# lean-dojo/ReProver

Hardware: NVIDIA H100
Metric: premises encoded/sec (reindex_corpus, ByT5-small, seq_len<=512) (higher is better)
Workload: dtype bf16

## Files before the change

### reprover_b200/csrc/rpx_encoder.cu

```cuda
#include <math.h>

#include <new>
#include <vector>

#include "rpx_gemm_launch.cuh"
#include "rpx_kernels.cuh"

namespace rpx {

namespace {

constexpr int kBlockN = 128;

struct LayerW {
  const __nv_bfloat16* qkv;
  const __nv_bfloat16* o;
  const __nv_bfloat16* wi;
  const __nv_bfloat16* wo;
};

struct ProfRec {
  int cls;
  cudaEvent_t a, b;
};
// ... 27 lines not shown
  const float* bias_lut = nullptr;
  std::vector<rpx::LayerW> layers;
  float* debug_hidden = nullptr;
  bool profiling = false;
  std::vector<rpx::ProfRec> prof_pending;
  std::vector<cudaEvent_t> event_pool;
  float prof_ms[RPX_N_KERNEL_CLASSES] = {0};
  int64_t prof_launches[RPX_N_KERNEL_CLASSES] = {0};
  std::vector<int32_t> h_cu_tokens;
  std::vector<int32_t> h_lens;
};

namespace rpx {

namespace {

struct PackedLayout {
  size_t emb, final_ln, bias_lut, bucket_tmp, layer0, layer_stride, qkv, o, wi, wo, total;
};

PackedLayout packed_layout(const rpx_t5_config& c) {
  PackedLayout L{};
  const size_t D = c.d_model, inner = (size_t)c.num_heads * c.d_kv, F = c.d_ff;
  size_t off = 0;
  auto take = [&](size_t bytes) {
    size_t o = off;
    off = align_up(off + bytes, 256);
    return o;
  };
  L.emb = take((size_t)c.vocab_size * D * 4);
  L.final_ln = take(D * 4);
  L.bias_lut = take((size_t)c.num_heads * (2 * c.rel_max_distance + 1) * 4);
  L.bucket_tmp = take((size_t)(2 * c.rel_max_distance + 1) * 4);
  L.layer0 = off;
  L.qkv = 0;
  size_t lo = 0;
  auto ltake = [&](size_t bytes) {
    size_t o = lo;
    lo = align_up(lo + bytes, 256);
    return o;
  };
  L.qkv = ltake(3 * inner * D * 2);
  L.o = ltake(D * inner * 2);
  L.wi = ltake(2 * F * D * 2);
  L.wo = ltake(D * F * 2);
  L.layer_stride = lo;
  L.total = L.layer0 + lo * (size_t)c.num_layers;
  return L;
}

int validate_cfg(const rpx_t5_config* c) {
  RPX_REQUIRE(c != nullptr, RPX_ERR_INVALID, "config is null");
  RPX_REQUIRE(c->d_kv == 64, RPX_ERR_UNSUPPORTED, "d_kv=%d: only 64 is implemented", c->d_kv);
  RPX_REQUIRE(c->d_model % 64 == 0 && c->d_model > 0, RPX_ERR_UNSUPPORTED, "d_model=%d must be a multiple of 64", c->d_model);
  RPX_REQUIRE(c->d_ff % 128 == 0 && c->d_ff > 0, RPX_ERR_UNSUPPORTED, "d_ff=%d must be a multiple of 128", c->d_ff);
  RPX_REQUIRE(c->num_heads > 0 && c->num_layers > 0 && c->vocab_size > 0, RPX_ERR_INVALID, "bad config");
  RPX_REQUIRE(c->rel_buckets >= 4 && c->rel_buckets % 4 == 0 && c->rel_max_distance >= c->rel_buckets / 4 &&
                  c->rel_max_distance <= 2048,
              RPX_ERR_UNSUPPORTED, "unsupported relative attention config (%d buckets, max distance %d)",
              c->rel_buckets, c->rel_max_distance);
  return RPX_OK;
}

__global__ void bias_lut_kernel(const float* __restrict__ rel_bias, const int32_t* __restrict__ buckets,
                                float* __restrict__ lut, int n_heads, int width) {
  const int i = blockIdx.x * blockDim.x + threadIdx.x;
  if (i >= n_heads * width) return;
  const int h = i / width, j = i % width;
  lut[i] = rel_bias[buckets[j] * n_heads + h];
}

struct Workspace {
  int32_t* cu_tokens;
  int64_t* cu_bytes;
  int32_t* ids;
  int32_t* lens;
  int32_t* flag;
  float* h32;
  __nv_bfloat16* h16;
  __nv_bfloat16* qkv;
  __nv_bfloat16* attn;
  __nv_bfloat16* ffn;
  float* ssA;
  float* ssB;
  size_t total;
};

Workspace carve(const rpx_encoder* e, uint8_t* base, int64_t T, int64_t S) {
  Workspace w{};
  const size_t D = e->cfg.d_model, inner = e->inner, F = e->cfg.d_ff;
  size_t off = 0;
  auto take = [&](size_t bytes) {
    uint8_t* p = base ? base + off : nullptr;
    off = align_up(off + bytes, 256);
    return p;
  };
  w.cu_tokens = (int32_t*)take((S + 1) * 4);
  w.cu_bytes = (int64_t*)take((S + 1) * 8);
  w.lens = (int32_t*)take((S + 1) * 4);
  w.flag = (int32_t*)take(256);
  w.ids = (int32_t*)take(T * 4);
  w.h32 = (float*)take(T * D * 4);
  w.h16 = (__nv_bfloat16*)take(T * D * 2);
  w.qkv = (__nv_bfloat16*)take(T * 3 * inner * 2);
  w.attn = (__nv_bfloat16*)take(T * inner * 2);
  w.ffn = (__nv_bfloat16*)take(T * F * 2);
  const size_t parts = e->n_parts > e->n_parts_lat ? e->n_parts : e->n_parts_lat;
  w.ssA = (float*)take(parts * T * 4);
  w.ssB = (float*)take(parts * T * 4);
  w.total = off;
  return w;
}

struct Prof {
  rpx_encoder* e;
  cudaStream_t st;
  int cls;
  cudaEvent_t a = nullptr, b = nullptr;
  Prof(rpx_encoder* e_, cudaStream_t st_, int cls_) : e(e_), st(st_), cls(cls_) {
    if (!e->profiling) return;
    a = get();
    b = get();
    cudaEventRecord(a, st);
  }
  ~Prof() {
    if (!e->profiling) return;
    cudaEventRecord(b, st);
    e->prof_pending.push_back({cls, a, b});
  }
  cudaEvent_t get() {
    if (!e->event_pool.empty()) {
      cudaEvent_t ev = e->event_pool.back();
      e->event_pool.pop_back();
      return ev;
    }
    cudaEvent_t ev;
    cudaEventCreate(&ev);
    return ev;
  }
};

constexpr int kLatBlockN = 64;
constexpr int kLatStages = 6;
constexpr int kLatSmallM = 64;
constexpr int kLatSmallStages = 12;
constexpr int kLatSmallMMaxTokens = 384;
constexpr int kPdlMaxTokens = 16384;

struct PdlScope {
  explicit PdlScope(bool on) { set_pdl_scope(on); }
  ~PdlScope() { set_pdl_scope(false); }
};

int ss_parts(int d_model, bool latency) {
  return ceil_div(d_model, latency ? 32 : kBlockN) * (EpiResidual::kWarps / 4);
}


int qkv_gemm(bool latency, int T, const void* A, const void* B, int N, int K, const RowScale& rs, __nv_bfloat16* out,
             const void* prefetch, size_t prefetch_bytes, cudaStream_t st) {
  EpiStoreBF16::Params ep{out, N, rs};
  if (!latency) return launch_gemm<kBlockN, EpiStoreBF16>(A, K, B, K, T, N, K, ep, st);
  if (T <= kLatSmallMMaxTokens)
    return launch_gemm<kLatBlockN, EpiStoreBF16, false, kLatSmallStages, false, kLatSmallM>(A, K, B, K, T, N, K, ep, st, 0,
                                                                                             prefetch, prefetch_bytes);
  return launch_gemm<kLatBlockN, EpiStoreBF16, false, kLatStages>(A, K, B, K, T, N, K, ep, st, 0, prefetch, prefetch_bytes);
}

int residual_gemm(bool latency, int T, const void* A, const void* B, int N, int K, float* h32, __nv_bfloat16* h16,
                  float* ss_out, cudaStream_t st) {
  EpiResidualParams ep{h32, h16, N, ss_out, T};
  if (!latency) return launch_gemm<kBlockN, EpiResidual>(A, K, B, K, T, N, K, ep, st);
  if (T <= kLatSmallMMaxTokens)
    return launch_gemm<kLatBlockN, EpiResidualT<true>, false, kLatSmallStages, false, kLatSmallM>(A, K, B, K, T, N, K, ep, st);
  return launch_gemm<kLatBlockN, EpiResidualT<true>, false, kLatStages>(A, K, B, K, T, N, K, ep, st);
}
int oproj_gemm(bool latency, int T, const void* A, const void* B, int N, int K, float* h32, __nv_bfloat16* h16,
               float* ss_out, cudaStream_t st) {
  return residual_gemm(latency, T, A, B, N, K, h32, h16, ss_out, st);
}
int ffn_down_gemm(bool latency, int T, const void* A, const void* B, int N, int K, float* h32, __nv_bfloat16* h16,
                  float* ss_out, cudaStream_t st) {
  return residual_gemm(latency, T, A, B, N, K, h32, h16, ss_out, st);
}

int ffn_up_gemm(bool latency, int T, const void* A, const void* B, int N, int K, const RowScale& rs,
                __nv_bfloat16* out, cudaStream_t st) {
  RPX_REQUIRE(N % 256 == 0, RPX_ERR_UNSUPPORTED, "ffn-up gemm: N=%d must be a multiple of 256 (2 x d_ff, d_ff %% 128 == 0)", N);
  const int F = N / 2;
  if (!latency) {
    EpiWsGeGLU::Params ep{out, F, rs};
    return launch_gemm_ws<EpiWsGeGLU>(A, K, B, K, T, N, K, ep, st);
  }
  if (T <= kBlockM) {
    EpiGeGLUT<32>::Params ep{out, F, rs};
    return launch_gemm<64, EpiGeGLUT<32>, false, kLatStages, true>(A, K, B, K, T, N, K, ep, st);
  }
  EpiGeGLUT<64>::Params ep{out, F, rs};
  return launch_gemm<128, EpiGeGLUT<64>, false, kGemmStages, true>(A, K, B, K, T, N, K, ep, st);
}

int forward_latency_layer(rpx_encoder* e, const Workspace& ws, const LayerW& w, const void* next_weights,
                          size_t next_bytes, int T, int S, int max_len, cudaStream_t st) {
  const rpx_t5_config& c = e->cfg;
  const int D = c.d_model, inner = e->inner, F = c.d_ff, P = e->n_parts_lat;
  const float inv_d = 1.0f / (float)D;
  {
    Prof p(e, st, 1);
    RPX_TRY(qkv_gemm(true, T, ws.h16, w.qkv, 3 * inner, D, RowScale{ws.ssA, P, T, inv_d, c.ln_eps}, ws.qkv, next_weights,
                     next_bytes, st));
  }
  {
    Prof p(e, st, 2);
    RPX_TRY(launch_t5_attention(ws.qkv, ws.attn, ws.cu_tokens, e->bias_lut, T, S, max_len, c.num_heads, c.d_kv,
                                c.rel_max_distance, st));
  }
  {
    Prof p(e, st, 3);
    RPX_TRY(oproj_gemm(true, T, ws.attn, w.o, D, inner, ws.h32, ws.h16, ws.ssB, st));
  }
  {
    Prof p(e, st, 4);
    RPX_TRY(ffn_up_gemm(true, T, ws.h16, w.wi, 2 * F, D, RowScale{ws.ssB, P, T, inv_d, c.ln_eps}, ws.ffn, st));
  }
  {
    Prof p(e, st, 5);
    RPX_TRY(ffn_down_gemm(true, T, ws.ffn, w.wo, D, F, ws.h32, ws.h16, ws.ssA, st));
  }
  return RPX_OK;
}

int forward(rpx_encoder* e, const Workspace& ws, int T, int S, int max_len, void* d_out, int out_dtype,
            cudaStream_t st) {
  const rpx_t5_config& c = e->cfg;
  const int D = c.d_model, inner = e->inner, F = c.d_ff;
  const bool latency = T <= e->latency_tokens && D % 32 == 0 && (3 * inner) % 32 == 0;
  const int P = latency ? e->n_parts_lat : e->n_parts;
  const float inv_d = 1.0f / (float)D;
  PdlScope pdl_scope(latency || T <= kPdlMaxTokens);
  {
    Prof p(e, st, 0);
    RPX_TRY(launch_embed(ws.ids, e->emb, ws.h32, ws.h16, ws.ssA, T, P, T, D, st));
  }
  auto dump = [&](int slab) -> int {
    if (e->debug_hidden)
      RPX_CUDA_OK(cudaMemcpyAsync(e->debug_hidden + (size_t)slab * T * D, ws.h32, (size_t)T * D * 4,
                                  cudaMemcpyDeviceToDevice, st));
    return RPX_OK;
  };
  RPX_TRY(dump(0));
  for (int l = 0; l < c.num_layers; ++l) {
    const LayerW& w = e->layers[l];
    if (latency) {
      const bool has_next = l + 1 < c.num_layers;
      RPX_TRY(forward_latency_layer(e, ws, w, has_next ? e->layers[l + 1].qkv : nullptr, has_next ? e->layer_bytes : 0, T, S,
                                    max_len, st));
      RPX_TRY(dump(l + 1));
      continue;
    }
    {
      Prof p(e, st, 1);
      RPX_TRY(qkv_gemm(false, T, ws.h16, w.qkv, 3 * inner, D, RowScale{ws.ssA, P, T, inv_d, c.ln_eps}, ws.qkv, nullptr, 0,
                       st));
    }
    {
      Prof p(e, st, 2);
      RPX_TRY(launch_t5_attention(ws.qkv, ws.attn, ws.cu_tokens, e->bias_lut, T, S, max_len, c.num_heads, c.d_kv,
                                  c.rel_max_distance, st));
    }
    {
      Prof p(e, st, 3);
      RPX_TRY(oproj_gemm(false, T, ws.attn, w.o, D, inner, ws.h32, ws.h16, ws.ssB, st));
    }
    {
      Prof p(e, st, 4);
      RPX_TRY(ffn_up_gemm(false, T, ws.h16, w.wi, 2 * F, D, RowScale{ws.ssB, P, T, inv_d, c.ln_eps}, ws.ffn, st));
    }
    {
      Prof p(e, st, 5);
      RPX_TRY(ffn_down_gemm(false, T, ws.ffn, w.wo, D, F, ws.h32, ws.h16, ws.ssA, st));
    }
    RPX_TRY(dump(l + 1));
  }
  {
    Prof p(e, st, 6);
    float* scratch = latency && (size_t)F * 2 >= (size_t)D * 4 ? reinterpret_cast<float*>(ws.ffn) : nullptr;
    RPX_TRY(launch_pool_normalize(ws.h32, ws.ssA, T, P, e->final_ln, ws.cu_tokens, d_out, out_dtype, S, D,
                                  c.ln_eps, st, scratch, max_len));
  }
  return RPX_OK;
}

}
}

using namespace rpx;

extern "C" {

size_t rpx_encoder_packed_bytes(const rpx_t5_config* cfg) {
  if (validate_cfg(cfg) != RPX_OK) return 0;
  return packed_layout(*cfg).total;
}

int rpx_encoder_create(const rpx_t5_config* cfg, const rpx_t5_weights* w, void* d_packed, size_t packed_bytes,
                       void* stream, rpx_encoder** out) {
  RPX_TRY(validate_cfg(cfg));
  RPX_REQUIRE(w && d_packed && out, RPX_ERR_INVALID, "rpx_encoder_create: null argument");
  DeviceInfo dev;
  RPX_TRY(get_device_info(&dev));
  const PackedLayout L = packed_layout(*cfg);
  RPX_REQUIRE(packed_bytes >= L.total, RPX_ERR_WORKSPACE, "packed buffer too small: %zu < %zu", packed_bytes, L.total);
  RPX_REQUIRE((reinterpret_cast<uintptr_t>(d_packed) & 255) == 0, RPX_ERR_INVALID, "packed buffer must be 256-byte aligned");
  cudaStream_t st = static_cast<cudaStream_t>(stream);
  uint8_t* base = static_cast<uint8_t*>(d_packed);
  const int D = cfg->d_model, inner = cfg->num_heads * cfg->d_kv, F = cfg->d_ff;

  rpx_encoder* e = new (std::nothrow) rpx_encoder();
  RPX_REQUIRE(e != nullptr, RPX_ERR_INVALID, "out of host memory");
  e->cfg = *cfg;
  e->inner = inner;
  e->n_parts = ss_parts(D, false);
  e->n_parts_lat = ss_parts(D, true);
  auto fail = [&](int code) {
    delete e;
    return code;
  };
#define TRY_E(expr)                        \
  do {                                     \
    int _s = (expr);                       \
    if (_s != RPX_OK) return fail(_s);     \
  } while (0)
#define CUDA_E(expr)                                                                                   \
  do {                                                                                                 \
    cudaError_t _c = (expr);                                                                           \
    if (_c != cudaSuccess) {                                                                           \
// ... 206 lines not shown
```

### reprover_b200/csrc/rpx_gemm.cuh

```cuda
#pragma once
#include "rpx_ptx.cuh"

namespace rpx {

constexpr int kBlockM = 128;
constexpr int kBlockK = 64;
constexpr int kMmaK = 16;
#ifndef RPX_EPI_WARPS
#define RPX_EPI_WARPS 4
#endif
constexpr int kMmaThreads = 128;
constexpr int kProducerWarp = 4;
constexpr int kEpiWarp0 = 5;
template <class Epi>
constexpr int gemm_threads() { return kMmaThreads + 32 + 32 * Epi::kWarps; }

template <int BLOCK_N, int STAGES, int BM = kBlockM>
struct GemmCfg {
  static_assert(BM == 64 || BM == 128, "tile rows: one or two 64-row wgmma blocks");
  static_assert(BLOCK_N == 64 || BLOCK_N == 128, "wgmma N of a tile: 64 or 128");
  static_assert(2 * STAGES + 2 <= 30, "barrier block holds at most 14 stages");
  static constexpr int kABytes = BM * kBlockK * 2;
  static constexpr int kBBytes = BLOCK_N * kBlockK * 2;
  static constexpr int kStageBytes = kABytes + kBBytes;
// ... 221 lines not shown
      }
      mbar_arrive(tfull);
      tphase ^= 1;
    }
  } else {
    const int lane_grp = (warp - kEpiWarp0) & 3;
    const int lane = threadIdx.x & 31;
    const int row = BM == kBlockM ? lane_grp * 32 + lane : (lane < 16 ? lane_grp * 16 + lane : (1 << 28));
    const int acc_row = BM == kBlockM ? lane_grp * 32 + lane : lane_grp * 16 + (lane & 15);
    const int part = (warp - kEpiWarp0) >> 2;
    pdl_wait();
    Epi epi(ep, smem_extra, lane_grp * 32 + lane, part);
    uint32_t tphase = 0;
    for (int u = unit0; u < num_units; u += unit_step) {
      TileCtx t;
      t.n_blk = unit_n(u);
      t.m_blk = unit_m(u);
      t.m0 = t.m_blk * BM;
      t.rows_per_warp = BM / 4;
      t.n0 = t.n_blk * n_blk_stride * BLOCK_N;
      int n_this = N - t.n0;
      if (n_this > BLOCK_N) n_this = BLOCK_N;
      t.n_cols = n_this;
      t.row = row;
      t.part = part;
      t.split = Epi::kWarps / 4;
      t.M = M;
      t.N = N;
      t.acc = sAcc + acc_row * Cfg::kAccStride;
      {
        const int nu = u + unit_step;
        if (nu < num_units) {
          t.next_m0 = unit_m(nu) * BM;
          t.next_n0 = unit_n(nu) * BLOCK_N;
          t.next_cols = N - t.next_n0 < BLOCK_N ? N - t.next_n0 : BLOCK_N;
        } else {
          t.next_m0 = -1;
          t.next_n0 = 0;
          t.next_cols = 0;
        }
      }
      epi.before_wait(t);
      mbar_wait(tfull, tphase);
      if (threadIdx.x == 32 * kEpiWarp0 && u == unit0) RPX_STAMP(pf, 5);
      epi.tile(t);
      if (threadIdx.x == 32 * kEpiWarp0 && u == unit0) RPX_STAMP(pf, 6);
      mbar_arrive(tempty);
      tphase ^= 1;
    }
    epi.finish();
  }

  __syncthreads();
  if (PAIR) cluster_sync_all();
  if (threadIdx.x == 0) RPX_STAMP(pf, 7);
}


struct RowScale {
  const float* ss_parts;
  int n_parts;
  int part_stride;
  float inv_dim;
  float eps;
  __device__ float get(int m) const {
    if (ss_parts == nullptr) return 1.0f;
    float s = 0.f;
    constexpr int kBatch = 24;
    for (int p = 0; p < n_parts; p += kBatch) {
      float v[kBatch];
#pragma unroll
      for (int j = 0; j < kBatch; ++j) v[j] = p + j < n_parts ? ss_parts[(size_t)(p + j) * part_stride + m] : 0.f;
#pragma unroll
      for (int j = 0; j < kBatch; ++j)
        if (p + j < n_parts) s += v[j];
    }
    return rsqrtf(s * inv_dim + eps);
  }
};

struct EpiStoreF32 {
  struct Params {
    float* C;
    int ldc;
  };
  static constexpr size_t kSmemBytes = 0;
  static constexpr int kWarps = RPX_EPI_WARPS;
  Params p;
  __device__ EpiStoreF32(const Params& p_, uint8_t*, int, int) : p(p_) {}
  __device__ void before_wait(const TileCtx&) {}
  __device__ void tile(const TileCtx& t) {
    const int m = t.m0 + t.row;
    const bool ok = m < t.M;
    for (int c = 32 * t.part; c < t.n_cols; c += 32 * t.split) {
      uint32_t v[32];
      acc_ld32(t.acc + c, v);
      if (ok) {
        float4* dst = reinterpret_cast<float4*>(p.C + (size_t)m * p.ldc + t.n0 + c);
#pragma unroll
        for (int i = 0; i < 8; ++i)
          dst[i] = make_float4(__uint_as_float(v[4 * i]), __uint_as_float(v[4 * i + 1]),
                               __uint_as_float(v[4 * i + 2]), __uint_as_float(v[4 * i + 3]));
      }
    }
  }
  __device__ void finish() {}
};

struct EpiStoreBF16 {
  struct Params {
    __nv_bfloat16* C;
    int ldc;
    RowScale rs;
  };
  static constexpr size_t kSmemBytes = 0;
  static constexpr int kWarps = RPX_EPI_WARPS;
  Params p;
  float rs = 0.f;
  __device__ EpiStoreBF16(const Params& p_, uint8_t*, int, int) : p(p_) {}
  __device__ void before_wait(const TileCtx& t) {
    const int m = t.m0 + t.row;
    rs = m < t.M ? p.rs.get(m) : 0.f;
  }
  __device__ void tile(const TileCtx& t) {
    const int m = t.m0 + t.row;
    const bool ok = m < t.M;
    for (int c = 32 * t.part; c < t.n_cols; c += 32 * t.split) {
      uint32_t v[32];
      acc_ld32(t.acc + c, v);
      if (ok) {
        uint4* dst = reinterpret_cast<uint4*>(p.C + (size_t)m * p.ldc + t.n0 + c);
#pragma unroll
        for (int i = 0; i < 4; ++i) {
          uint4 o;
          o.x = pack_bf16x2(__uint_as_float(v[8 * i + 0]) * rs, __uint_as_float(v[8 * i + 1]) * rs);
          o.y = pack_bf16x2(__uint_as_float(v[8 * i + 2]) * rs, __uint_as_float(v[8 * i + 3]) * rs);
          o.z = pack_bf16x2(__uint_as_float(v[8 * i + 4]) * rs, __uint_as_float(v[8 * i + 5]) * rs);
          o.w = pack_bf16x2(__uint_as_float(v[8 * i + 6]) * rs, __uint_as_float(v[8 * i + 7]) * rs);
          dst[i] = o;
        }
      }
    }
  }
  __device__ void finish() {}
};

struct EpiResidualParams {
  float* h32;
  __nv_bfloat16* h16;
  int ld;
  float* ss_out;
  int ss_stride;
};
template <bool CHUNK_SS>
struct EpiResidualT {
  using Params = EpiResidualParams;
  static constexpr int kWarps = RPX_EPI_WARPS;
  static constexpr size_t kSmemBytes = kWarps * 32 * 32 * sizeof(float);
  Params p;
  float4* stg;
  int lane, grp;
  float4 h[8];
  __device__ EpiResidualT(const Params& p_, uint8_t* smem_extra, int row, int part) : p(p_) {
    lane = row & 31;
    grp = row >> 5;
    stg = reinterpret_cast<float4*>(smem_extra) + (part * 4 + grp) * 32 * 8;
  }
  __device__ __forceinline__ void load_chunk(const TileCtx& t, int c, int row_base, int sub, int col4,
                                             float4 (&hh)[8]) const {
    const size_t col = (size_t)t.n0 + c + col4;
#pragma unroll
    for (int i = 0; i < 8; ++i) {
      const int r = sub + 4 * i, m = row_base + r;
      if (r < t.rows_per_warp && m < t.M) hh[i] = *reinterpret_cast<const float4*>(p.h32 + (size_t)m * p.ld + col);
      else hh[i] = make_float4(0.f, 0.f, 0.f, 0.f);
    }
  }
  __device__ void before_wait(const TileCtx& t) {
    const int c = 32 * t.part;
    if (c < t.n_cols) load_chunk(t, c, t.m0 + grp * t.rows_per_warp, lane >> 3, (lane & 7) * 4, h);
  }
  __device__ void tile(const TileCtx& t) {
    const int sub = lane >> 3;
    const int j4 = lane & 7;
    const int col4 = j4 * 4;
    const int row_base = t.m0 + grp * t.rows_per_warp;
    const int step = 32 * t.split;
    float ss[8];
#pragma unroll
    for (int i = 0; i < 8; ++i) ss[i] = 0.f;
    float4 hn[8];
    int c = 32 * t.part;
    for (; c < t.n_cols; c += step) {
      uint32_t v[32];
      acc_ld32(t.acc + c, v);
      if (c + step < t.n_cols) load_chunk(t, c + step, row_base, sub, col4, hn);
      const size_t col = (size_t)t.n0 + c + col4;
#pragma unroll
      for (int j = 0; j < 8; ++j)
        stg[lane * 8 + (j ^ (lane & 7))] =
            make_float4(__uint_as_float(v[4 * j]), __uint_as_float(v[4 * j + 1]), __uint_as_float(v[4 * j + 2]),
                        __uint_as_float(v[4 * j + 3]));
      __syncwarp();
#pragma unroll
      for (int i = 0; i < 8; ++i) {
        const int r = sub + 4 * i;
        const int m = row_base + r;
        const float4 a = stg[r * 8 + (j4 ^ (r & 7))];
        h[i].x += a.x;
        h[i].y += a.y;
        h[i].z += a.z;
        h[i].w += a.w;
        ss[i] += h[i].x * h[i].x + h[i].y * h[i].y + h[i].z * h[i].z + h[i].w * h[i].w;
        if (r < t.rows_per_warp && m < t.M) {
          *reinterpret_cast<float4*>(p.h32 + (size_t)m * p.ld + col) = h[i];
          *reinterpret_cast<uint2*>(p.h16 + (size_t)m * p.ld + col) =
              make_uint2(pack_bf16x2(h[i].x, h[i].y), pack_bf16x2(h[i].z, h[i].w));
        }
      }
      __syncwarp();
#pragma unroll
      for (int i = 0; i < 8; ++i) h[i] = hn[i];
      if (CHUNK_SS) {
        write_ss(t, ss, row_base, sub, (t.n0 + c) >> 5);
#pragma unroll
        for (int i = 0; i < 8; ++i) ss[i] = 0.f;
      }
    }
    if (!CHUNK_SS) write_ss(t, ss, row_base, sub, t.n_blk * t.split + t.part);
  }
  __device__ __forceinline__ void write_ss(const TileCtx& t, float (&ss)[8], int row_base, int sub, int part_idx) const {
#pragma unroll
    for (int i = 0; i < 8; ++i) {
      float v = ss[i];
      v += __shfl_xor_sync(0xffffffffu, v, 1);
      v += __shfl_xor_sync(0xffffffffu, v, 2);
      v += __shfl_xor_sync(0xffffffffu, v, 4);
      const int r = sub + 4 * i, m = row_base + r;
      if ((lane & 7) == 0 && r < t.rows_per_warp && m < t.M) p.ss_out[(size_t)part_idx * p.ss_stride + m] = v;
    }
  }
  __device__ void finish() {}
};
using EpiResidual = EpiResidualT<false>;

__device__ __forceinline__ float gelu_new(float x) {
  const float k0 = 0.7978845608028654f;
  const float k1 = 0.044715f;
  float u = k0 * (x + k1 * x * x * x);
  float t;
  asm("tanh.approx.f32 %0, %1;" : "=f"(t) : "f"(u));
  return 0.5f * x * (1.0f + t);
}

template <int HALF>
struct EpiGeGLUT {
  struct Params {
    __nv_bfloat16* out;
    int ldo;
    RowScale rs;
  };
  static constexpr size_t kSmemBytes = 0;
  static constexpr int kWarps = RPX_EPI_WARPS;
  Params p;
  float rs = 0.f;
  __device__ EpiGeGLUT(const Params& p_, uint8_t*, int, int) : p(p_) {}
  __device__ void before_wait(const TileCtx& t) {
    const int m = t.m0 + t.row;
    rs = m < t.M ? p.rs.get(m) : 0.f;
  }
  __device__ void tile(const TileCtx& t) {
    const int m = t.m0 + t.row;
    const bool ok = m < t.M;
    for (int c = 32 * t.part; c < HALF; c += 32 * t.split) {
      uint32_t g[32], u[32];
      acc_ld32(t.acc + c, g);
      acc_ld32(t.acc + HALF + c, u);
      if (ok) {
        uint4* dst = reinterpret_cast<uint4*>(p.out + (size_t)m * p.ldo + t.n_blk * HALF + c);
#pragma unroll
        for (int i = 0; i < 4; ++i) {
          float r[8];
#pragma unroll
          for (int j = 0; j < 8; ++j)
            r[j] = gelu_new(__uint_as_float(g[8 * i + j]) * rs) * (__uint_as_float(u[8 * i + j]) * rs);
          uint4 o;
          o.x = pack_bf16x2(r[0], r[1]);
          o.y = pack_bf16x2(r[2], r[3]);
          o.z = pack_bf16x2(r[4], r[5]);
          o.w = pack_bf16x2(r[6], r[7]);
          dst[i] = o;
        }
      }
    }
  }
  __device__ void finish() {}
};

}
```

### reprover_b200/csrc/rpx_gemm_launch.cuh

```cuda
#pragma once
#include "rpx_common.cuh"
#include "rpx_gemm.cuh"
#include "rpx_gemm_ws.cuh"

namespace rpx {

constexpr int kGemmStages = 4;

template <int BLOCK_N, class Epi, bool M_FASTEST = false, int STAGES = kGemmStages, bool SPLIT_B = false, int BM = kBlockM>
int launch_gemm(const void* A, int64_t lda, const void* B, int64_t ldb, int M, int N, int K,
                const typename Epi::Params& ep, cudaStream_t stream, int grid_limit = 0, const void* prefetch_ptr = nullptr,
                size_t prefetch_bytes = 0) {
  using Cfg = GemmCfg<BLOCK_N, STAGES, BM>;
  static_assert(BM == kBlockM || (!M_FASTEST && Epi::kWarps == 4), "64-row tiles: encoder epilogues with one warp per lane group");
  RPX_REQUIRE(M > 0 && N > 0 && K > 0, RPX_ERR_INVALID, "gemm: empty problem M=%d N=%d K=%d", M, N, K);
  RPX_REQUIRE(K % kBlockK == 0, RPX_ERR_UNSUPPORTED, "gemm: K=%d must be a multiple of %d", K, kBlockK);
  RPX_REQUIRE(M_FASTEST || N % 32 == 0, RPX_ERR_UNSUPPORTED, "gemm: N=%d must be a multiple of 32", N);
  DeviceInfo dev;
  RPX_TRY(get_device_info(&dev));
  CUtensorMap tmA, tmB;
  RPX_TRY(make_tmap_bf16_2d(&tmA, A, (uint64_t)M, (uint64_t)K, (uint64_t)lda, BM));
  RPX_TRY(make_tmap_bf16_2d(&tmB, B, (uint64_t)N, (uint64_t)K, (uint64_t)ldb, SPLIT_B ? BLOCK_N / 2 : BLOCK_N));
  RPX_REQUIRE(!SPLIT_B || N % BLOCK_N == 0, RPX_ERR_UNSUPPORTED, "gemm: split-B tiles need N %% %d == 0", BLOCK_N);
  const int tiles_m = ceil_div(M, BM);
  const int tiles_n = ceil_div(N, BLOCK_N);
  const size_t smem = Cfg::smem_bytes(Epi::kSmemBytes);
  RPX_REQUIRE(smem <= dev.smem_optin, RPX_ERR_UNSUPPORTED, "gemm: needs %zu B smem, device allows %zu",
              smem, dev.smem_optin);
  auto kern = gemm_tc_kernel<BLOCK_N, STAGES, Epi, M_FASTEST, SPLIT_B, BM>;
  static thread_local int configured_dev = -1;
  if (configured_dev != dev.device) {
    RPX_CUDA_OK(cudaFuncSetAttribute(kern, cudaFuncAttributeMaxDynamicSharedMemorySize, (int)smem));
    configured_dev = dev.device;
  }
  int grid = tiles_m * tiles_n;
  int cap = grid_limit > 0 ? grid_limit : dev.num_sms;
  if (grid > cap) grid = cap;
  L2Prefetch pf{prefetch_ptr, (uint32_t)prefetch_bytes, grid, next_timeline_slot()};
  if (prefetch_ptr != nullptr && prefetch_bytes > 0 && prefetch_bytes < ((size_t)1 << 32) && grid < dev.num_sms)
    grid = dev.num_sms;
  RPX_CUDA_OK(launch_pdl(kern, dim3(grid), dim3(gemm_threads<Epi>()), smem, stream, pdl_enabled(), tmA, tmB, M, N, K, tiles_m,
                         tiles_n, 1, ep, pf));
  return RPX_OK;
}

template <class Epi>
int launch_gemm_ws(const void* A, int64_t lda, const void* B, int64_t ldb, int M, int N, int K,
                   const typename Epi::Params& ep, cudaStream_t stream) {
  RPX_REQUIRE(M > 0 && N > 0 && K > 0, RPX_ERR_INVALID, "gemm: empty problem M=%d N=%d K=%d", M, N, K);
  RPX_REQUIRE(K % kBlockK == 0, RPX_ERR_UNSUPPORTED, "gemm: K=%d must be a multiple of %d", K, kBlockK);
  RPX_REQUIRE(N % 32 == 0, RPX_ERR_UNSUPPORTED, "gemm: N=%d must be a multiple of 32", N);
  DeviceInfo dev;
  RPX_TRY(get_device_info(&dev));
  CUtensorMap tmA, tmB;
  RPX_TRY(make_tmap_bf16_2d(&tmA, A, (uint64_t)M, (uint64_t)K, (uint64_t)lda, kBlockM));
  RPX_TRY(make_tmap_bf16_2d(&tmB, B, (uint64_t)N, (uint64_t)K, (uint64_t)ldb, kWsBlockN));
  const int tiles_m = ceil_div(M, kBlockM);
  const int tiles_n = ceil_div(N, kWsBlockN);
  const size_t smem = WsCfg::kSmemBytes;
  RPX_REQUIRE(smem <= dev.smem_optin, RPX_ERR_UNSUPPORTED, "gemm: needs %zu B smem, device allows %zu", smem,
              dev.smem_optin);
  auto kern = gemm_ws_kernel<Epi>;
  static thread_local int configured_dev = -1;
  if (configured_dev != dev.device) {
    RPX_CUDA_OK(cudaFuncSetAttribute(kern, cudaFuncAttributeMaxDynamicSharedMemorySize, (int)smem));
    configured_dev = dev.device;
  }
  int grid = tiles_m * tiles_n;
  if (grid > dev.num_sms) grid = dev.num_sms;
  RPX_CUDA_OK(launch_pdl(kern, dim3(grid), dim3(kWsThreads), smem, stream, pdl_enabled(), tmA, tmB, M, N, K, tiles_m,
                         tiles_n, ep));
  return RPX_OK;
}

template <class Epi, int STAGES = kGemmStages>
int launch_gemm_pair(const void* A, int64_t lda, const void* B, int64_t ldb, int M, int N, int K,
                     const typename Epi::Params& ep, cudaStream_t stream) {
  constexpr int BLOCK_N = 128;
  using Cfg = GemmCfg<BLOCK_N, STAGES, kBlockM>;
  RPX_REQUIRE(M > 0 && N > 0 && K > 0, RPX_ERR_INVALID, "gemm: empty problem M=%d N=%d K=%d", M, N, K);
  RPX_REQUIRE(K % kBlockK == 0, RPX_ERR_UNSUPPORTED, "gemm: K=%d must be a multiple of %d", K, kBlockK);
  RPX_REQUIRE(N % 32 == 0, RPX_ERR_UNSUPPORTED, "gemm: N=%d must be a multiple of 32", N);
  DeviceInfo dev;
  RPX_TRY(get_device_info(&dev));
  CUtensorMap tmA, tmB;
  RPX_TRY(make_tmap_bf16_2d(&tmA, A, (uint64_t)M, (uint64_t)K, (uint64_t)lda, kBlockM));
  RPX_TRY(make_tmap_bf16_2d(&tmB, B, (uint64_t)N, (uint64_t)K, (uint64_t)ldb, BLOCK_N / 2));
  const int tiles_m = ceil_div(M, kBlockM);
  const int tiles_n = ceil_div(N, BLOCK_N);
  const size_t smem = Cfg::smem_bytes(Epi::kSmemBytes);
  RPX_REQUIRE(smem <= dev.smem_optin, RPX_ERR_UNSUPPORTED, "gemm: needs %zu B smem, device allows %zu", smem,
              dev.smem_optin);
  auto kern = gemm_tc_kernel<BLOCK_N, STAGES, Epi, false, false, kBlockM, true>;
  static thread_local int configured_dev = -1;
  if (configured_dev != dev.device) {
    RPX_CUDA_OK(cudaFuncSetAttribute(kern, cudaFuncAttributeMaxDynamicSharedMemorySize, (int)smem));
    configured_dev = dev.device;
  }
  int pairs = ceil_div(tiles_m, 2) * tiles_n;
  if (pairs > dev.num_sms / 2) pairs = dev.num_sms / 2;
  cudaLaunchConfig_t cfg{};
  cfg.gridDim = dim3(2 * pairs);
  cfg.blockDim = dim3(gemm_threads<Epi>());
  cfg.dynamicSmemBytes = smem;
  cfg.stream = stream;
  cudaLaunchAttribute at[1];
  at[0].id = cudaLaunchAttributeClusterDimension;
  at[0].val.clusterDim.x = 2;
  at[0].val.clusterDim.y = 1;
  at[0].val.clusterDim.z = 1;
  cfg.attrs = at;
  cfg.numAttrs = 1;
  RPX_CUDA_OK(cudaLaunchKernelEx(&cfg, kern, tmA, tmB, M, N, K, tiles_m, tiles_n, 1, ep,
                                 L2Prefetch{nullptr, 0u, 2 * pairs, next_timeline_slot()}));
  return RPX_OK;
}

}
```

### reprover_b200/csrc/rpx_gemm_ws.cuh

```cuda
#pragma once
#include "rpx_gemm.cuh"

namespace rpx {

constexpr int kWsBlockN = 256;
constexpr int kWsStages = 4;
constexpr int kWsThreads = 384;

struct WsCfg {
  static constexpr int kABytes = kBlockM * kBlockK * 2;
  static constexpr int kBBytes = kWsBlockN * kBlockK * 2;
  static constexpr int kStageBytes = kABytes + kBBytes;
  static constexpr size_t kSmemBytes = (size_t)kWsStages * kStageBytes + 1024 + 256;
};

struct FragCtx {
  int m0, n0;
  int n_blk;
  int n_cols;
  int M, N;
  int r0;
  int q;
};

template <class Epi>
__global__ void __launch_bounds__(kWsThreads, 1)
gemm_ws_kernel(const __grid_constant__ CUtensorMap tmA, const __grid_constant__ CUtensorMap tmB, int M, int N, int K,
               int tiles_m, int tiles_n, typename Epi::Params ep) {
  extern __shared__ uint8_t smem_raw[];
  const uint32_t raw_addr = smem_u32(smem_raw);
  uint8_t* smem = smem_raw + ((1024 - (raw_addr & 1023)) & 1023);
  uint8_t* sA = smem;
  uint8_t* sB = smem + kWsStages * WsCfg::kABytes;
  uint64_t* full = reinterpret_cast<uint64_t*>(smem + kWsStages * WsCfg::kStageBytes);
  uint64_t* empty = full + kWsStages;

  const int warp = threadIdx.x >> 5;
  const int wg = warp >> 2;
  const int num_kb = K / kBlockK;
  const int num_tiles = tiles_m * tiles_n;

  if (threadIdx.x == 0) {
    tma_prefetch_desc(&tmA);
    tma_prefetch_desc(&tmB);
    for (int s = 0; s < kWsStages; ++s) {
      mbar_init(&full[s], 1);
      mbar_init(&empty[s], 2 * 128);
    }
    fence_mbar_init();
  }
  __syncthreads();
  pdl_launch_dependents();
  pdl_wait();

  if (wg == 0) {
    setmaxnreg_dec<40>();
    if (warp == 0 && elect_one()) {
      int stage = 0;
      uint32_t phase = 0;
      for (int t = blockIdx.x; t < num_tiles; t += gridDim.x) {
        const int m_blk = t / tiles_n, n_blk = t % tiles_n;
        for (int kb = 0; kb < num_kb; ++kb) {
          mbar_wait(&empty[stage], phase ^ 1);
          mbar_arrive_expect_tx(&full[stage], WsCfg::kStageBytes);
          tma_load_2d(sA + stage * WsCfg::kABytes, &tmA, &full[stage], kb * kBlockK, m_blk * kBlockM);
          tma_load_2d(sB + stage * WsCfg::kBBytes, &tmB, &full[stage], kb * kBlockK, n_blk * kWsBlockN);
          if (++stage == kWsStages) {
            stage = 0;
            phase ^= 1;
          }
        }
      }
    }
  } else {
    setmaxnreg_inc<232>();
    const int cw = wg - 1;
    const int lane = threadIdx.x & 31;
    Epi epi(ep);
    float acc[128];
    int stage = 0;
    uint32_t phase = 0;
    for (int t = blockIdx.x; t < num_tiles; t += gridDim.x) {
      FragCtx c;
      c.n_blk = t % tiles_n;
      c.m0 = (t / tiles_n) * kBlockM;
      c.n0 = c.n_blk * kWsBlockN;
      c.n_cols = N - c.n0 < kWsBlockN ? N - c.n0 : kWsBlockN;
      c.M = M;
      c.N = N;
      c.r0 = c.m0 + 64 * cw + 16 * (warp & 3) + (lane >> 2);
      c.q = lane & 3;
      int prev = 0;
      for (int kb = 0; kb < num_kb; ++kb) {
        mbar_wait(&full[stage], phase);
        const uint64_t a_desc = make_smem_desc_kmajor_sw128(smem_u32(sA + stage * WsCfg::kABytes)) + 512 * cw;
        const uint64_t b_desc = make_smem_desc_kmajor_sw128(smem_u32(sB + stage * WsCfg::kBBytes));
        wgmma_fence_operand(acc);
        wgmma_fence();
#pragma unroll
        for (int k = 0; k < kBlockK / kMmaK; ++k) wgmma_m64n256k16_ss(acc, a_desc + 2 * k, b_desc + 2 * k, (kb | k) != 0);
        wgmma_commit();
        if (kb == 0) epi.prefetch(c);
        if (kb > 0) {
          wgmma_wait<1>();
          mbar_arrive(&empty[prev]);
        }
        prev = stage;
        if (++stage == kWsStages) {
          stage = 0;
          phase ^= 1;
        }
      }
      wgmma_wait<0>();
      wgmma_fence_operand(acc);
      mbar_arrive(&empty[prev]);
      epi.tile(c, acc);
    }
  }
}


struct EpiWsStoreF32 {
  using Params = EpiStoreF32::Params;
  Params p;
  __device__ explicit EpiWsStoreF32(const Params& p_) : p(p_) {}
  __device__ void prefetch(const FragCtx&) {}
  __device__ void tile(const FragCtx& c, const float (&acc)[128]) {
#pragma unroll
    for (int j = 0; j < 32; ++j) {
      if (8 * j < c.n_cols) {
        float* dst = p.C + (size_t)c.r0 * p.ldc + c.n0 + 8 * j + 2 * c.q;
        if (c.r0 < c.M) *reinterpret_cast<float2*>(dst) = make_float2(acc[4 * j], acc[4 * j + 1]);
        if (c.r0 + 8 < c.M) *reinterpret_cast<float2*>(dst + 8 * (size_t)p.ldc) = make_float2(acc[4 * j + 2], acc[4 * j + 3]);
      }
    }
  }
};

struct EpiWsGeGLU {
  struct Params {
    __nv_bfloat16* out;
    int ldo;
    RowScale rs;
  };
  Params p;
  float rs0 = 0.f, rs1 = 0.f;
  __device__ explicit EpiWsGeGLU(const Params& p_) : p(p_) {}
  __device__ void prefetch(const FragCtx& c) {
    rs0 = c.r0 < c.M ? p.rs.get(c.r0) : 0.f;
    rs1 = c.r0 + 8 < c.M ? p.rs.get(c.r0 + 8) : 0.f;
  }
  __device__ void tile(const FragCtx& c, const float (&acc)[128]) {
    __nv_bfloat16* dst = p.out + (size_t)c.r0 * p.ldo + c.n_blk * (kWsBlockN / 2) + 2 * c.q;
#pragma unroll
    for (int j = 0; j < 16; ++j) {
      const float* g = acc + 4 * j;
      const float* u = acc + 4 * (j + 16);
      if (c.r0 < c.M)
        *reinterpret_cast<uint32_t*>(dst + 8 * j) =
            pack_bf16x2(gelu_new(g[0] * rs0) * (u[0] * rs0), gelu_new(g[1] * rs0) * (u[1] * rs0));
      if (c.r0 + 8 < c.M)
        *reinterpret_cast<uint32_t*>(dst + 8 * (size_t)p.ldo + 8 * j) =
            pack_bf16x2(gelu_new(g[2] * rs1) * (u[2] * rs1), gelu_new(g[3] * rs1) * (u[3] * rs1));
    }
  }
};

}
```

Measured before the change: 3026.

## Route throughput residual GEMMs through warp-specialized kernel with TMA-streamed residual epilogue

Moves the non-latency o-proj and FFN-down residual GEMMs from the classic 128-wide kernel to the persistent warp-specialized 256-wide wgmma kernel. Two idle producer-group warps now stream the fp32 residual in 64x32 chunks via TMA into a small smem ring, and the consumer warpgroups add the accumulator in place, write fp32/bf16 outputs and per-128-column sum-of-squares. Stage count becomes a template parameter, tuned separately per GEMM against the residual buffers. This trades smem and barrier complexity for overlapping residual loads with the MMA mainloop and larger tiles.

```diff
diff --git a/reprover_b200/csrc/rpx_encoder.cu b/reprover_b200/csrc/rpx_encoder.cu
--- a/reprover_b200/csrc/rpx_encoder.cu
+++ b/reprover_b200/csrc/rpx_encoder.cu
@@ -203,9 +203,7 @@
   ~PdlScope() { set_pdl_scope(false); }
 };
 
-int ss_parts(int d_model, bool latency) {
-  return ceil_div(d_model, latency ? 32 : kBlockN) * (EpiResidual::kWarps / 4);
-}
+int ss_parts(int d_model, bool latency) { return ceil_div(d_model, latency ? 32 : 128); }
 
 
 int qkv_gemm(bool latency, int T, const void* A, const void* B, int N, int K, const RowScale& rs, __nv_bfloat16* out,
@@ -218,21 +216,22 @@
   return launch_gemm<kLatBlockN, EpiStoreBF16, false, kLatStages>(A, K, B, K, T, N, K, ep, st, 0, prefetch, prefetch_bytes);
 }
 
+template <int RES_BUFS, int STAGES>
 int residual_gemm(bool latency, int T, const void* A, const void* B, int N, int K, float* h32, __nv_bfloat16* h16,
                   float* ss_out, cudaStream_t st) {
   EpiResidualParams ep{h32, h16, N, ss_out, T};
-  if (!latency) return launch_gemm<kBlockN, EpiResidual>(A, K, B, K, T, N, K, ep, st);
+  if (!latency) return launch_gemm_ws<EpiWsResidual<RES_BUFS>, STAGES>(A, K, B, K, T, N, K, ep, st);
   if (T <= kLatSmallMMaxTokens)
-    return launch_gemm<kLatBlockN, EpiResidualT<true>, false, kLatSmallStages, false, kLatSmallM>(A, K, B, K, T, N, K, ep, st);
-  return launch_gemm<kLatBlockN, EpiResidualT<true>, false, kLatStages>(A, K, B, K, T, N, K, ep, st);
+    return launch_gemm<kLatBlockN, EpiResidualChunkSS, false, kLatSmallStages, false, kLatSmallM>(A, K, B, K, T, N, K, ep, st);
+  return launch_gemm<kLatBlockN, EpiResidualChunkSS, false, kLatStages>(A, K, B, K, T, N, K, ep, st);
 }
 int oproj_gemm(bool latency, int T, const void* A, const void* B, int N, int K, float* h32, __nv_bfloat16* h16,
                float* ss_out, cudaStream_t st) {
-  return residual_gemm(latency, T, A, B, N, K, h32, h16, ss_out, st);
+  return residual_gemm<2, 4>(latency, T, A, B, N, K, h32, h16, ss_out, st);
 }
 int ffn_down_gemm(bool latency, int T, const void* A, const void* B, int N, int K, float* h32, __nv_bfloat16* h16,
                   float* ss_out, cudaStream_t st) {
-  return residual_gemm(latency, T, A, B, N, K, h32, h16, ss_out, st);
+  return residual_gemm<5, 3>(latency, T, A, B, N, K, h32, h16, ss_out, st);
 }
 
 int ffn_up_gemm(bool latency, int T, const void* A, const void* B, int N, int K, const RowScale& rs,
diff --git a/reprover_b200/csrc/rpx_gemm.cuh b/reprover_b200/csrc/rpx_gemm.cuh
--- a/reprover_b200/csrc/rpx_gemm.cuh
+++ b/reprover_b200/csrc/rpx_gemm.cuh
@@ -397,8 +397,7 @@
   float* ss_out;
   int ss_stride;
 };
-template <bool CHUNK_SS>
-struct EpiResidualT {
+struct EpiResidualChunkSS {
   using Params = EpiResidualParams;
   static constexpr int kWarps = RPX_EPI_WARPS;
   static constexpr size_t kSmemBytes = kWarps * 32 * 32 * sizeof(float);
@@ -406,7 +405,7 @@
   float4* stg;
   int lane, grp;
   float4 h[8];
-  __device__ EpiResidualT(const Params& p_, uint8_t* smem_extra, int row, int part) : p(p_) {
+  __device__ EpiResidualChunkSS(const Params& p_, uint8_t* smem_extra, int row, int part) : p(p_) {
     lane = row & 31;
     grp = row >> 5;
     stg = reinterpret_cast<float4*>(smem_extra) + (part * 4 + grp) * 32 * 8;
@@ -466,13 +465,10 @@
       __syncwarp();
 #pragma unroll
       for (int i = 0; i < 8; ++i) h[i] = hn[i];
-      if (CHUNK_SS) {
-        write_ss(t, ss, row_base, sub, (t.n0 + c) >> 5);
-#pragma unroll
-        for (int i = 0; i < 8; ++i) ss[i] = 0.f;
-      }
-    }
-    if (!CHUNK_SS) write_ss(t, ss, row_base, sub, t.n_blk * t.split + t.part);
+      write_ss(t, ss, row_base, sub, (t.n0 + c) >> 5);
+#pragma unroll
+      for (int i = 0; i < 8; ++i) ss[i] = 0.f;
+    }
   }
   __device__ __forceinline__ void write_ss(const TileCtx& t, float (&ss)[8], int row_base, int sub, int part_idx) const {
 #pragma unroll
@@ -487,7 +483,6 @@
   }
   __device__ void finish() {}
 };
-using EpiResidual = EpiResidualT<false>;
 
 __device__ __forceinline__ float gelu_new(float x) {
   const float k0 = 0.7978845608028654f;
diff --git a/reprover_b200/csrc/rpx_gemm_launch.cuh b/reprover_b200/csrc/rpx_gemm_launch.cuh
--- a/reprover_b200/csrc/rpx_gemm_launch.cuh
+++ b/reprover_b200/csrc/rpx_gemm_launch.cuh
@@ -44,7 +44,7 @@
   return RPX_OK;
 }
 
-template <class Epi>
+template <class Epi, int STAGES = 4>
 int launch_gemm_ws(const void* A, int64_t lda, const void* B, int64_t ldb, int M, int N, int K,
                    const typename Epi::Params& ep, cudaStream_t stream) {
   RPX_REQUIRE(M > 0 && N > 0 && K > 0, RPX_ERR_INVALID, "gemm: empty problem M=%d N=%d K=%d", M, N, K);
@@ -52,15 +52,19 @@
   RPX_REQUIRE(N % 32 == 0, RPX_ERR_UNSUPPORTED, "gemm: N=%d must be a multiple of 32", N);
   DeviceInfo dev;
   RPX_TRY(get_device_info(&dev));
-  CUtensorMap tmA, tmB;
+  CUtensorMap tmA, tmB, tmR;
   RPX_TRY(make_tmap_bf16_2d(&tmA, A, (uint64_t)M, (uint64_t)K, (uint64_t)lda, kBlockM));
   RPX_TRY(make_tmap_bf16_2d(&tmB, B, (uint64_t)N, (uint64_t)K, (uint64_t)ldb, kWsBlockN));
+  if constexpr (Epi::kResBufs > 0)
+    RPX_TRY(make_tmap_2d(&tmR, 4, ep.h32, (uint64_t)M, (uint64_t)N, (uint64_t)ep.ld, kResChunkCols, 64, 128));
+  else
+    tmR = tmA;
   const int tiles_m = ceil_div(M, kBlockM);
   const int tiles_n = ceil_div(N, kWsBlockN);
-  const size_t smem = WsCfg::kSmemBytes;
+  const size_t smem = WsCfg<STAGES, Epi::kResBufs>::kSmemBytes;
   RPX_REQUIRE(smem <= dev.smem_optin, RPX_ERR_UNSUPPORTED, "gemm: needs %zu B smem, device allows %zu", smem,
               dev.smem_optin);
-  auto kern = gemm_ws_kernel<Epi>;
+  auto kern = gemm_ws_kernel<Epi, STAGES>;
   static thread_local int configured_dev = -1;
   if (configured_dev != dev.device) {
     RPX_CUDA_OK(cudaFuncSetAttribute(kern, cudaFuncAttributeMaxDynamicSharedMemorySize, (int)smem));
@@ -68,8 +72,8 @@
   }
   int grid = tiles_m * tiles_n;
   if (grid > dev.num_sms) grid = dev.num_sms;
-  RPX_CUDA_OK(launch_pdl(kern, dim3(grid), dim3(kWsThreads), smem, stream, pdl_enabled(), tmA, tmB, M, N, K, tiles_m,
-                         tiles_n, ep));
+  RPX_CUDA_OK(launch_pdl(kern, dim3(grid), dim3(kWsThreads), smem, stream, pdl_enabled(), tmA, tmB, tmR, M, N, K,
+                         tiles_m, tiles_n, ep));
   return RPX_OK;
 }
 
diff --git a/reprover_b200/csrc/rpx_gemm_ws.cuh b/reprover_b200/csrc/rpx_gemm_ws.cuh
--- a/reprover_b200/csrc/rpx_gemm_ws.cuh
+++ b/reprover_b200/csrc/rpx_gemm_ws.cuh
@@ -4,14 +4,19 @@
 namespace rpx {
 
 constexpr int kWsBlockN = 256;
-constexpr int kWsStages = 4;
 constexpr int kWsThreads = 384;
-
+constexpr int kResChunkCols = 32;
+constexpr int kResChunkBytes = 64 * kResChunkCols * 4;
+
+template <int STAGES, int RES_BUFS>
 struct WsCfg {
+  static_assert(2 * STAGES + 4 * RES_BUFS <= 32, "barrier block holds 32 mbarriers");
   static constexpr int kABytes = kBlockM * kBlockK * 2;
   static constexpr int kBBytes = kWsBlockN * kBlockK * 2;
   static constexpr int kStageBytes = kABytes + kBBytes;
-  static constexpr size_t kSmemBytes = (size_t)kWsStages * kStageBytes + 1024 + 256;
+  static constexpr int kRingBytes = STAGES * kStageBytes;
+  static constexpr int kResBytes = 2 * RES_BUFS * kResChunkBytes;
+  static constexpr size_t kSmemBytes = (size_t)kRingBytes + kResBytes + 1024 + 256;
 };
 
 struct FragCtx {
@@ -23,17 +28,29 @@
   int q;
 };
 
-template <class Epi>
+struct ResStream {
+  float* buf;
+  uint64_t* full;
+  uint64_t* empty;
+};
+
+template <class Epi, int STAGES>
 __global__ void __launch_bounds__(kWsThreads, 1)
-gemm_ws_kernel(const __grid_constant__ CUtensorMap tmA, const __grid_constant__ CUtensorMap tmB, int M, int N, int K,
-               int tiles_m, int tiles_n, typename Epi::Params ep) {
+gemm_ws_kernel(const __grid_constant__ CUtensorMap tmA, const __grid_constant__ CUtensorMap tmB,
+               const __grid_constant__ CUtensorMap tmR, int M, int N, int K, int tiles_m, int tiles_n,
+               typename Epi::Params ep) {
+  using Cfg = WsCfg<STAGES, Epi::kResBufs>;
+  constexpr int R = Epi::kResBufs;
   extern __shared__ uint8_t smem_raw[];
   const uint32_t raw_addr = smem_u32(smem_raw);
   uint8_t* smem = smem_raw + ((1024 - (raw_addr & 1023)) & 1023);
   uint8_t* sA = smem;
-  uint8_t* sB = smem + kWsStages * WsCfg::kABytes;
-  uint64_t* full = reinterpret_cast<uint64_t*>(smem + kWsStages * WsCfg::kStageBytes);
-  uint64_t* empty = full + kWsStages;
+  uint8_t* sB = smem + STAGES * Cfg::kABytes;
+  float* sR = reinterpret_cast<float*>(smem + Cfg::kRingBytes);
+  uint64_t* full = reinterpret_cast<uint64_t*>(smem + Cfg::kRingBytes + Cfg::kResBytes);
+  uint64_t* empty = full + STAGES;
+  uint64_t* rfull = empty + STAGES;
+  uint64_t* rempty = rfull + 2 * R;
 
   const int warp = threadIdx.x >> 5;
   const int wg = warp >> 2;
@@ -43,9 +60,14 @@
   if (threadIdx.x == 0) {
     tma_prefetch_desc(&tmA);
     tma_prefetch_desc(&tmB);
-    for (int s = 0; s < kWsStages; ++s) {
+    if (R > 0) tma_prefetch_desc(&tmR);
+    for (int s = 0; s < STAGES; ++s) {
       mbar_init(&full[s], 1);
       mbar_init(&empty[s], 2 * 128);
+    }
+    for (int s = 0; s < 2 * R; ++s) {
+      mbar_init(&rfull[s], 1);
+      mbar_init(&rempty[s], 128);
     }
     fence_mbar_init();
   }
@@ -62,11 +84,33 @@
         const int m_blk = t / tiles_n, n_blk = t % tiles_n;
         for (int kb = 0; kb < num_kb; ++kb) {
           mbar_wait(&empty[stage], phase ^ 1);
-          mbar_arrive_expect_tx(&full[stage], WsCfg::kStageBytes);
-          tma_load_2d(sA + stage * WsCfg::kABytes, &tmA, &full[stage], kb * kBlockK, m_blk * kBlockM);
-          tma_load_2d(sB + stage * WsCfg::kBBytes, &tmB, &full[stage], kb * kBlockK, n_blk * kWsBlockN);
-          if (++stage == kWsStages) {
+          mbar_arrive_expect_tx(&full[stage], Cfg::kStageBytes);
+          tma_load_2d(sA + stage * Cfg::kABytes, &tmA, &full[stage], kb * kBlockK, m_blk * kBlockM);
+          tma_load_2d(sB + stage * Cfg::kBBytes, &tmB, &full[stage], kb * kBlockK, n_blk * kWsBlockN);
+          if (++stage == STAGES) {
             stage = 0;
+            phase ^= 1;
+          }
+        }
+      }
+    } else if (R > 0 && (warp == 1 || warp == 2) && elect_one()) {
+      const int w = warp - 1;
+      float* buf = sR + w * R * (kResChunkBytes / 4);
+      uint64_t* rf = rfull + w * R;
+      uint64_t* re = rempty + w * R;
+      int b = 0;
+      uint32_t phase = 0;
+      for (int t = blockIdx.x; t < num_tiles; t += gridDim.x) {
+        const int row0 = (t / tiles_n) * kBlockM + 64 * w;
+        const int n0 = (t % tiles_n) * kWsBlockN;
+        const int n_cols = N - n0 < kWsBlockN ? N - n0 : kWsBlockN;
+        if (row0 >= M) continue;
+        for (int col = 0; col < n_cols; col += kResChunkCols) {
+          mbar_wait(&re[b], phase ^ 1);
+          mbar_arrive_expect_tx(&rf[b], kResChunkBytes);
+          tma_load_2d(buf + b * (kResChunkBytes / 4), &tmR, &rf[b], n0 + col, row0);
+          if (++b == R) {
+            b = 0;
             phase ^= 1;
           }
         }
@@ -76,7 +120,7 @@
     setmaxnreg_inc<232>();
     const int cw = wg - 1;
     const int lane = threadIdx.x & 31;
-    Epi epi(ep);
+    Epi epi(ep, ResStream{sR + cw * R * (kResChunkBytes / 4), rfull + cw * R, rempty + cw * R});
     float acc[128];
     int stage = 0;
     uint32_t phase = 0;
@@ -93,8 +137,8 @@
       int prev = 0;
       for (int kb = 0; kb < num_kb; ++kb) {
         mbar_wait(&full[stage], phase);
-        const uint64_t a_desc = make_smem_desc_kmajor_sw128(smem_u32(sA + stage * WsCfg::kABytes)) + 512 * cw;
-        const uint64_t b_desc = make_smem_desc_kmajor_sw128(smem_u32(sB + stage * WsCfg::kBBytes));
+        const uint64_t a_desc = make_smem_desc_kmajor_sw128(smem_u32(sA + stage * Cfg::kABytes)) + 512 * cw;
+        const uint64_t b_desc = make_smem_desc_kmajor_sw128(smem_u32(sB + stage * Cfg::kBBytes));
         wgmma_fence_operand(acc);
         wgmma_fence();
 #pragma unroll
@@ -106,7 +150,7 @@
           mbar_arrive(&empty[prev]);
         }
         prev = stage;
-        if (++stage == kWsStages) {
+        if (++stage == STAGES) {
           stage = 0;
           phase ^= 1;
         }
@@ -122,8 +166,9 @@
 
 struct EpiWsStoreF32 {
   using Params = EpiStoreF32::Params;
+  static constexpr int kResBufs = 0;
   Params p;
-  __device__ explicit EpiWsStoreF32(const Params& p_) : p(p_) {}
+  __device__ EpiWsStoreF32(const Params& p_, const ResStream&) : p(p_) {}
   __device__ void prefetch(const FragCtx&) {}
   __device__ void tile(const FragCtx& c, const float (&acc)[128]) {
 #pragma unroll
@@ -143,9 +188,10 @@
     int ldo;
     RowScale rs;
   };
+  static constexpr int kResBufs = 0;
   Params p;
   float rs0 = 0.f, rs1 = 0.f;
-  __device__ explicit EpiWsGeGLU(const Params& p_) : p(p_) {}
+  __device__ EpiWsGeGLU(const Params& p_, const ResStream&) : p(p_) {}
   __device__ void prefetch(const FragCtx& c) {
     rs0 = c.r0 < c.M ? p.rs.get(c.r0) : 0.f;
     rs1 = c.r0 + 8 < c.M ? p.rs.get(c.r0 + 8) : 0.f;
@@ -166,4 +212,79 @@
   }
 };
 
+template <int RES_BUFS>
+struct EpiWsResidual {
+  using Params = EpiResidualParams;
+  static constexpr int kResBufs = RES_BUFS;
+  Params p;
+  ResStream rs;
+  int b = 0;
+  uint32_t phase = 0;
+  __device__ EpiWsResidual(const Params& p_, const ResStream& rs_) : p(p_), rs(rs_) {}
+  __device__ void prefetch(const FragCtx&) {}
+  __device__ void tile(const FragCtx& c, const float (&acc)[128]) {
+    const int lane = threadIdx.x & 31;
+    const int v = (threadIdx.x >> 5) & 3;
+    const int row0 = c.r0 - 16 * v - (lane >> 2);
+    if (row0 >= c.M) return;
+    const int sub = lane >> 3, j4 = lane & 7;
+    float ss[4];
+#pragma unroll
+    for (int k = 0; k < kWsBlockN / kResChunkCols; ++k) {
+      if (kResChunkCols * k >= c.n_cols) break;
+      if (k % 4 == 0) {
+#pragma unroll
+        for (int i = 0; i < 4; ++i) ss[i] = 0.f;
+      }
+      float* s = rs.buf + b * (kResChunkBytes / 4);
+      mbar_wait(&rs.full[b], phase);
+#pragma unroll
+      for (int jj = 0; jj < 4; ++jj) {
+        const int j = 4 * k + jj;
+#pragma unroll
+        for (int h = 0; h < 2; ++h) {
+          const int r = 16 * v + (lane >> 2) + 8 * h;
+          float2* x = reinterpret_cast<float2*>(s + r * kResChunkCols + (((2 * jj + (c.q >> 1)) ^ (r & 7)) << 2) + 2 * (c.q & 1));
+          float2 hv = *x;
+          hv.x += acc[4 * j + 2 * h];
+          hv.y += acc[4 * j + 2 * h + 1];
+          *x = hv;
+        }
+      }
+      __syncwarp();
+      const size_t col = (size_t)c.n0 + kResChunkCols * k + 4 * j4;
+#pragma unroll
+      for (int i = 0; i < 4; ++i) {
+        const int r = 16 * v + sub + 4 * i;
+        const int m = row0 + r;
+        const float4 hv = *reinterpret_cast<const float4*>(s + r * kResChunkCols + ((j4 ^ (r & 7)) << 2));
+        ss[i] += hv.x * hv.x + hv.y * hv.y + hv.z * hv.z + hv.w * hv.w;
+        if (m < c.M) {
+          *reinterpret_cast<float4*>(p.h32 + (size_t)m * p.ld + col) = hv;
+          *reinterpret_cast<uint2*>(p.h16 + (size_t)m * p.ld + col) =
+              make_uint2(pack_bf16x2(hv.x, hv.y), pack_bf16x2(hv.z, hv.w));
+        }
+      }
+      fence_proxy_async_smem();
+      mbar_arrive(&rs.empty[b]);
+      if (++b == RES_BUFS) {
+        b = 0;
+        phase ^= 1;
+      }
+      if (k % 4 == 3 || kResChunkCols * (k + 1) >= c.n_cols) {
+        const int part = 2 * c.n_blk + k / 4;
+#pragma unroll
+        for (int i = 0; i < 4; ++i) {
+          float t = ss[i];
+          t += __shfl_xor_sync(0xffffffffu, t, 1);
+          t += __shfl_xor_sync(0xffffffffu, t, 2);
+          t += __shfl_xor_sync(0xffffffffu, t, 4);
+          const int m = row0 + 16 * v + sub + 4 * i;
+          if (j4 == 0 && m < c.M) p.ss_out[(size_t)part * p.ss_stride + m] = t;
+        }
+      }
+    }
+  }
+};
+
 }
```

New measurement: 3168 (median of 6 runs). 1.05x the previous value.
